# LukasHaas/PIGEON

Hardware: AMD Instinct MI355X
Metric: images/sec end-to-end (ViT+head+refine), 4x336x336 (higher is better)
Workload: dtype f16

## Files before the change

### include/pigeon_hip.h

```cpp
#ifndef PIGEON_HIP_H
#define PIGEON_HIP_H

#include <stddef.h>
#include <stdint.h>

#ifdef __cplusplus
extern "C" {
#endif

#define PG_OK            0
#define PG_EINVAL       -1
#define PG_ENOMEM       -2
#define PG_EHIP         -3
#define PG_ESTATE       -4

#define PG_DTYPE_F32     0
#define PG_DTYPE_BF16    1
#define PG_DTYPE_F16     2
#define PG_DTYPE_F64     3
#define PG_DTYPE_U8      4

#define PG_ABI_VERSION   7

const char* pg_last_error(void);
// ... 97 lines not shown
                        float* tol, int32_t* code, void* stream);

int pg_refine_certainty_bank(const pg_bank* bank, const float* q, int B, int P, const int64_t* cand, const float* cand_prob, int k,
                             int topk, int n_eval, const float* scratch12, const float* W, int C, const float* beta,
                             const float* wstats, float temperature, const int32_t* refined, const int32_t* choice,
                             float* tol, int32_t* code, float bank_sigma, void* stream);

int pg_requeue_append(const float* head_tol, const float* refine_tol, const int32_t* refine_code, int B, float thr, int force_all,
                      int64_t dst_base, int64_t flushed, int64_t cap, int64_t* counters, int64_t* slot_dst, int32_t* row_slot,
                      uint8_t* certain, int32_t* cause, void* stream);
int pg_rows_to_slots(const void* src, int64_t row_bytes, const int32_t* row_slot, int B, void* dst, void* stream);
int pg_requeue_take(const int64_t* slot_dst, int64_t cap, int64_t head, int n_valid, int n_pad, int64_t* dst_out, void* stream);
int pg_scatter_rows(const void* src, int64_t row_bytes, const int64_t* dst_row, int n, void* dst, int64_t dst_rows,
                    int64_t remap_wb, int64_t remap_b, int64_t remap_off, void* stream);
int pg_head_wstats(const float* W, int C, const float* beta, float* out2, void* stream);

int pg_embedding_debias(float* emb, int64_t n, int dim, const float* bias, void* stream);

int pg_token_attribution(const float* hidden, int n_images, int P, const float* W, int C, const int64_t* cells,
                         const int64_t* against, int K, float* out, void* stream);

typedef struct pg_prep pg_prep;
int pg_prep_create(pg_prep** out, int device, int in_h, int in_w);
int pg_prep_destroy(pg_prep* h);
int pg_prep_geometry(const pg_prep* h, int32_t* out6);
int pg_prep_workspace_bytes(const pg_prep* h, int n_images, size_t* bytes);
int pg_prep_norm_lut(float out[768]);
int pg_prep_forward(pg_prep* h, const void* images_u8, int n_images, void* out, int out_dtype, void* workspace,
                    size_t workspace_bytes, void* stream);

// ... 110 lines not shown
int pg_op_gemm16_ld(int dtype, const void* A, int64_t lda, const void* W, int64_t ldw, const float* bias, void* out,
                    int64_t ldc, int M, int N, int K, int epi, float qscale, int qcols, const float* aux,
                    int variant, void* stream);
int pg_op_rowstat_cast(const float* x, void* x16, int dtype, float* rowstat, int64_t rows, float eps, void* stream);
int pg_op_gemm16_resid_stat(int dtype, const void* A, int64_t lda, const void* W, int64_t ldw, const float* bias, float* X,
                            int64_t ldc, void* x16, int64_t ldx, float* statpart, int M, int N, int K, int variant, void* stream);
int pg_op_rowstat_finalize(const float* statpart, int slots, float* rowstat, int64_t rows, float eps, void* stream);
int pg_op_gemm16_ln(int dtype, const void* A, int64_t lda, const void* W, int64_t ldw, const float* bias, const float* colsum,
                    const float* rowstat, void* out, int64_t ldc, int M, int N, int K, int epi, float qscale, int qcols,
                    int variant, void* stream);
int pg_op_layernorm(const float* x, const float* gamma, const float* beta, void* y, int out_dtype,
                    int64_t rows, float eps, void* stream);
int pg_op_attention(int dtype, const void* qkv, void* out, int n_images, void* stream);
int pg_op_im2col(const void* pixels, int pix_dtype, void* out, int out_dtype, int n_images, void* stream);
int pg_op_token_mean(const float* x, float* out, int n_images, void* stream);
int pg_op_cast_f32(const float* x, void* y, int out_dtype, int64_t n, void* stream);
int pg_op_preln(float* x, const float* cls, const float* pos0, const float* gamma, const float* beta, int64_t rows, float eps,
                void* x16, int x16_dtype, float* rowstat, void* stream);
int pg_op_gemm16_parts(int dtype, const void* A, int64_t lda, const void* W, int64_t ldw, const float* bias, float* parts,
                       int M, int N, int Kp, int S, void* stream);
int pg_op_x3_split(const float* x, void* y3, int64_t rows, int cols, int gelu, void* stream);
int pg_op_x3_layernorm(const float* x, const float* gamma, const float* beta, void* y3, int64_t rows, float eps, void* stream);
int pg_op_attention_f32(const float* qkv, float* out, int n_images, void* stream);
int pg_op_attention_x3(const float* qkv, void* out3, int n_images, void* stream);
int pg_op_x3_im2col(const void* pixels, int pix_dtype, void* out3, int n_images, void* stream);
int pg_op_sum_parts(const float* parts, int S, int64_t part_elems, float* dst, int64_t n, int resid, void* stream);

#ifdef __cplusplus
}
#endif
// ... 2 lines not shown
```

### pigeon_amd/_lib.py

```python
from __future__ import annotations

import ctypes as C
import os

_HERE = os.path.dirname(os.path.abspath(__file__))
LIB_PATH = os.environ.get("PIGEON_HIP_LIB") or os.path.join(_HERE, "libpigeon_hip.so")

PG_DTYPE_F32, PG_DTYPE_BF16, PG_DTYPE_F16, PG_DTYPE_F64, PG_DTYPE_U8 = 0, 1, 2, 3, 4
EPI_QKV, EPI_GELU, EPI_RESID, EPI_PATCH, EPI_F32, EPI_RESID_STAT, EPI_QKV_LN, EPI_GELU_LN, EPI_GELU_X3 = 0, 1, 2, 3, 4, 5, 6, 7, 8
PROF_CLASSES = ["gemm_qkv", "gemm_out", "gemm_fc1", "gemm_fc2", "gemm_patch", "attention", "layernorm",
                "im2col", "token_mean"]


class PigeonHipError(RuntimeError):
    pass


class VitCfg(C.Structure):
    _fields_ = [("layers", C.c_int32), ("image_size", C.c_int32), ("patch", C.c_int32), ("hidden", C.c_int32),
                ("heads", C.c_int32), ("mlp", C.c_int32), ("ln_eps", C.c_float), ("max_chunk", C.c_int32),
                ("mma_dtype", C.c_int32), ("precise", C.c_int32)]


class Bank(C.Structure):
# ... 19 lines not shown
PREP_ITEM_BYTES = 80
assert C.sizeof(PrepItem) == PREP_ITEM_BYTES


class JpegInfo(C.Structure):
    _fields_ = [("reason", C.c_int32), ("height", C.c_int32), ("width", C.c_int32), ("ncomp", C.c_int32), ("hs", C.c_int32),
                ("vs", C.c_int32), ("reserved", C.c_int32 * 2)]


class JpegItem(C.Structure):
    _fields_ = [("rgb_off", C.c_uint64), ("coef_off", C.c_uint64 * 3), ("plane_off", C.c_uint64 * 3), ("height", C.c_int32),
                ("width", C.c_int32), ("ncomp", C.c_int32), ("hs", C.c_int32), ("vs", C.c_int32), ("bw", C.c_int32 * 3),
                ("bh", C.c_int32 * 3), ("qsel", C.c_int32 * 3), ("reserved", C.c_int32 * 4), ("qt", (C.c_uint16 * 64) * 4)]


JPEG_ITEM_BYTES = 640
assert C.sizeof(JpegItem) == JPEG_ITEM_BYTES and C.sizeof(JpegInfo) == 32
JPEG_REASONS = ("ok", "not_jpeg", "progressive", "lossless", "hierarchical", "arithmetic", "precision", "components", "colorspace",
                "sampling", "multiscan", "dnl", "size", "malformed")


_P, _I, _I64, _F, _D, _SZ = C.c_void_p, C.c_int, C.c_int64, C.c_float, C.c_double, C.c_size_t
SIGNATURES = {
    "pg_last_error": (C.c_char_p, []),
    "pg_abi_version": (_I, []),
    "pg_device_count": (_I, []),
    "pg_vit_create": (_I, [C.POINTER(_P), _I, C.POINTER(VitCfg)]),
    "pg_vit_load_weight": (_I, [_P, C.c_char_p, _P, _I, C.POINTER(_I64), _I]),
    "pg_vit_finalize": (_I, [_P]),
    "pg_vit_workspace_bytes": (_I, [_P, _I, C.POINTER(_SZ)]),
# ... 59 lines not shown
    "pg_region_plan": (_I, [C.POINTER(RegionBankStruct), C.POINTER(C.c_int32)]),
    "pg_tune_region_wave_edges": (_I, [_I]),
    "pg_head_forward": (_I, [_P, _I, _I, _P, _P, _P, _I, _I, _P, _P, _P, _P, _P, _P]),
    "pg_head_margin": (_I, [_P, _I, _I, _P, _I, _P, _P, _P, _P, _P]),
    "pg_head_certainty": (_I, [_P, _I, _I, _P, _I, _P, _P, _I, _P, _P, _P, _P, _P, _P, _P]),
    "pg_aux_heads_forward": (_I, [_P, _I, _I, _P, _P, _I, _I, _I, _P, _P, _P, _P, _P, _P, _P]),
    "pg_refine_forward": (_I, [C.POINTER(Bank), _P, _I, _I, _P, _P, _P, _I, _I, _F, _D, _P, _P, _P, _P, _P]),
    "pg_refine_forward_ex": (_I, [C.POINTER(Bank), _P, _I, _I, _P, _P, _P, _I, _I, _I, _F, _D, _P, _P, _P, _P, _P, _P]),
    "pg_refine_certainty": (_I, [C.POINTER(Bank), _P, _I, _I, _P, _P, _I, _I, _I, _P, _P, _I, _P, _P, _F, _P, _P, _P, _P, _P]),
    "pg_refine_certainty_bank": (_I, [C.POINTER(Bank), _P, _I, _I, _P, _P, _I, _I, _I, _P, _P, _I, _P, _P, _F, _P, _P, _P, _P, _F, _P]),
    "pg_requeue_append": (_I, [_P, _P, _P, _I, _F, _I, _I64, _I64, _I64, _P, _P, _P, _P, _P, _P]),
    "pg_rows_to_slots": (_I, [_P, _I64, _P, _I, _P, _P]),
    "pg_requeue_take": (_I, [_P, _I64, _I64, _I, _I, _P, _P]),
    "pg_scatter_rows": (_I, [_P, _I64, _P, _I, _P, _I64, _I64, _I64, _I64, _P]),
    "pg_head_wstats": (_I, [_P, _I, _P, _P, _P]),
    "pg_embedding_debias": (_I, [_P, _I64, _I, _P, _P]),
    "pg_token_attribution": (_I, [_P, _I, _I, _P, _I, _P, _P, _I, _P, _P]),
    "pg_op_gemm16": (_I, [_I, _P, _I64, _P, _P, _P, _I64, _I, _I, _I, _I, _F, _I, _P, _I, _P]),
    "pg_op_gemm16_ld": (_I, [_I, _P, _I64, _P, _I64, _P, _P, _I64, _I, _I, _I, _I, _F, _I, _P, _I, _P]),
    "pg_op_rowstat_cast": (_I, [_P, _P, _I, _P, _I64, _F, _P]),
    "pg_op_gemm16_resid_stat": (_I, [_I, _P, _I64, _P, _I64, _P, _P, _I64, _P, _I64, _P, _I, _I, _I, _I, _P]),
    "pg_op_rowstat_finalize": (_I, [_P, _I, _P, _I64, _F, _P]),
    "pg_op_gemm16_ln": (_I, [_I, _P, _I64, _P, _I64, _P, _P, _P, _P, _I64, _I, _I, _I, _I, _F, _I, _I, _P]),
    "pg_op_layernorm": (_I, [_P, _P, _P, _P, _I, _I64, _F, _P]),
    "pg_op_attention": (_I, [_I, _P, _P, _I, _P]),
    "pg_op_im2col": (_I, [_P, _I, _P, _I, _I, _P]),
    "pg_op_token_mean": (_I, [_P, _P, _I, _P]),
    "pg_op_cast_f32": (_I, [_P, _P, _I, _I64, _P]),
    "pg_op_gemm16_parts": (_I, [_I, _P, _I64, _P, _I64, _P, _P, _I, _I, _I, _I, _P]),
    "pg_op_x3_split": (_I, [_P, _P, _I64, _I, _I, _P]),
    "pg_op_x3_layernorm": (_I, [_P, _P, _P, _P, _I64, _F, _P]),
    "pg_op_attention_f32": (_I, [_P, _P, _I, _P]),
    "pg_op_attention_x3": (_I, [_P, _P, _I, _P]),
    "pg_op_x3_im2col": (_I, [_P, _I, _P, _I, _P]),
    "pg_op_sum_parts": (_I, [_P, _I, _I64, _P, _I64, _I, _P]),
    "pg_op_preln": (_I, [_P, _P, _P, _P, _P, _I64, _F, _P, _I, _P, _P]),
    "pg_vit_precise_plan": (_I, [_I, C.POINTER(C.c_int32)]),
}

_lib = None


# ... 32 lines not shown
```

### pigeon_amd/csrc/abi.hip

```cpp
#include "pigeon_internal.h"
#include <cstdarg>
#include <cstdio>

static thread_local char g_err[512] = "";

void pg_set_error(const char* fmt, ...) {
    va_list ap;
    va_start(ap, fmt);
    vsnprintf(g_err, sizeof(g_err), fmt, ap);
    va_end(ap);
}
int pg_check_launch(const char* what) {
    hipError_t e = hipGetLastError();
    if (e != hipSuccess) { pg_set_error("launch of %s failed: %s", what, hipGetErrorString(e)); return PG_EHIP; }
    return PG_OK;
}

extern "C" const char* pg_last_error(void) { return g_err; }
extern "C" int pg_abi_version(void) { return PG_ABI_VERSION; }
extern "C" int pg_device_count(void) {
    int n = 0;
    hipError_t e = hipGetDeviceCount(&n);
    if (e != hipSuccess) { pg_set_error("hipGetDeviceCount: %s", hipGetErrorString(e)); return PG_EHIP; }
    return n;
// ... 44 lines not shown
extern "C" int pg_op_attention(int dtype, const void* qkv, void* out, int n_images, void* stream) {
    if (!qkv || !out) { pg_set_error("op_attention: null argument"); return PG_EINVAL; }
    return pg_attention_launch(dtype, qkv, out, n_images, (hipStream_t)stream);
}
extern "C" int pg_op_im2col(const void* pixels, int pix_dtype, void* out, int out_dtype, int n_images, void* stream) {
    if (!pixels || !out) { pg_set_error("op_im2col: null argument"); return PG_EINVAL; }
    if (out_dtype == PG_DTYPE_U8) { pg_set_error("op_im2col: PG_DTYPE_U8 is a pixel dtype, not an output dtype"); return PG_EINVAL; }
    const float* lut = nullptr;
    if (pix_dtype == PG_DTYPE_U8 && n_images > 0) { const int rc = pg_norm_lut_device(&lut); if (rc) return rc; }
    return pg_im2col_launch(pixels, pix_dtype, out, out_dtype, n_images, (hipStream_t)stream, lut);
}
extern "C" int pg_op_token_mean(const float* x, float* out, int n_images, void* stream) {
    if (!x || !out) { pg_set_error("op_token_mean: null argument"); return PG_EINVAL; }
    return pg_token_mean_launch(x, out, n_images, (hipStream_t)stream);
}
extern "C" int pg_op_cast_f32(const float* x, void* y, int out_dtype, int64_t n, void* stream) {
    if (!x || !y) { pg_set_error("op_cast_f32: null argument"); return PG_EINVAL; }
    return pg_cast_f32_launch(x, y, out_dtype, n, (hipStream_t)stream);
}

extern "C" int pg_op_gemm16_parts(int dtype, const void* A, int64_t lda, const void* W, int64_t ldw, const float* bias, float* parts,
                                  int M, int N, int Kp, int S, void* stream) {
    if (!A || !W || !parts) { pg_set_error("op_gemm16_parts: null argument"); return PG_EINVAL; }
    if (S < 1 || S > 8) { pg_set_error("op_gemm16_parts: 1 <= S <= 8"); return PG_EINVAL; }
    PgGemmExtra ex;
    ex.parts = S; ex.a_part = Kp; ex.w_part = Kp; ex.c_part = (int64_t)M * N;
    return pg_gemm_launch(dtype, A, lda, W, ldw, bias, parts, N, M, N, Kp, EPI_F32, 1.f, 0, nullptr, PG_GEMM_V_PP, (hipStream_t)stream, &ex);
}

extern "C" int pg_op_x3_split(const float* x, void* y3, int64_t rows, int cols, int gelu, void* stream) {
// ... 33 lines not shown
```

### pigeon_amd/csrc/comm.hip

```cpp
#include "pigeon_internal.h"

#include <dlfcn.h>
#include <unistd.h>
#include <cstdio>
#include <cstdlib>
#include <cstring>
#include <rccl/rccl.h>

namespace {

struct Rccl {
    void* lib = nullptr;
    ncclResult_t (*GetUniqueId)(ncclUniqueId*) = nullptr;
    ncclResult_t (*CommInitRank)(ncclComm_t*, int, ncclUniqueId, int) = nullptr;
    ncclResult_t (*CommDestroy)(ncclComm_t) = nullptr;
    ncclResult_t (*CommCount)(const ncclComm_t, int*) = nullptr;
    ncclResult_t (*AllGather)(const void*, void*, size_t, ncclDataType_t, ncclComm_t, hipStream_t) = nullptr;
    ncclResult_t (*GroupStart)() = nullptr;
    ncclResult_t (*GroupEnd)() = nullptr;
    const char* (*GetErrorString)(ncclResult_t) = nullptr;
    ncclResult_t (*GetVersion)(int*) = nullptr;
};

Rccl* rccl() {
// ... 85 lines not shown
    if (!R) return PG_EHIP;
    pg_comm* c = (pg_comm*)comm;
    PG_NCCL(R->AllGather(send, recv, bytes_per_rank, ncclInt8, c->comm, (hipStream_t)stream));
    return PG_OK;
}

extern "C" int pg_allgather_many(void* comm, int count, const void* const* send, void* const* recv, const size_t* bytes_per_rank,
                                 void* stream) {
    if (!comm || count < 0 || (count > 0 && (!send || !recv || !bytes_per_rank))) { pg_set_error("allgather_many: bad argument"); return PG_EINVAL; }
    if (count == 0) return PG_OK;
    Rccl* R = rccl();
    if (!R) return PG_EHIP;
    pg_comm* c = (pg_comm*)comm;
    for (int i = 0; i < count; ++i)
        if (bytes_per_rank[i] && (!send[i] || !recv[i])) { pg_set_error("allgather_many: null buffer %d", i); return PG_EINVAL; }
    PG_NCCL(R->GroupStart());
    ncclResult_t first = ncclSuccess;
    for (int i = 0; i < count; ++i) {
        if (!bytes_per_rank[i]) continue;
        const ncclResult_t e = R->AllGather(send[i], recv[i], bytes_per_rank[i], ncclInt8, c->comm, (hipStream_t)stream);
        if (e != ncclSuccess && first == ncclSuccess) first = e;
    }
    const ncclResult_t e2 = R->GroupEnd();
    if (first != ncclSuccess) { pg_set_error("ncclAllGather (grouped) failed: %s", R->GetErrorString(first)); return PG_EHIP; }
    if (e2 != ncclSuccess) { pg_set_error("ncclGroupEnd failed: %s", R->GetErrorString(e2)); return PG_EHIP; }
    return PG_OK;
}

extern "C" int pg_comm_destroy(void* comm) {
    if (!comm) return PG_OK;
// ... 15 lines not shown
```

### pigeon_amd/csrc/head.hip

```cpp
#include "common.h"
#include "pigeon_internal.h"
#include "certainty_common.h"
#include <cfloat>

#define HT 64
#define HK 32

__global__ __launch_bounds__(256) void head_logits_kernel(const float* __restrict__ emb, int B, int P,
                                                          const float* __restrict__ W, const float* __restrict__ bias,
                                                          int C, float* __restrict__ logits) {
    __shared__ float As[HK][HT + 1];
    __shared__ float Ws[HK][HT + 1];
    const int tid = threadIdx.x;
    const int c0 = blockIdx.x * HT, b0 = blockIdx.y * HT;
    const int tx = tid & 15, ty = tid >> 4;
    float acc[4][4];
#pragma unroll
    for (int i = 0; i < 4; ++i)
#pragma unroll
        for (int j = 0; j < 4; ++j) acc[i][j] = 0.f;
    const float invP = 1.0f / (float)P;
    for (int k0 = 0; k0 < VIT_HIDDEN; k0 += HK) {
#pragma unroll
        for (int i = 0; i < 8; ++i) {
            const int idx = tid + i * 256;
// ... 20 lines not shown
#pragma unroll
                for (int j = 0; j < 4; ++j) acc[i][j] = fmaf(a[i], w[j], acc[i][j]);
        }
        __syncthreads();
    }
#pragma unroll
    for (int i = 0; i < 4; ++i) {
        const int b = b0 + ty * 4 + i;
        if (b >= B) continue;
#pragma unroll
        for (int j = 0; j < 4; ++j) {
            const int c = c0 + tx * 4 + j;
            if (c < C) logits[(int64_t)b * C + c] = acc[i][j] + bias[c];
        }
    }
}

struct ValIdx { float v; int i; };
__device__ __forceinline__ ValIdx block_argbest(ValIdx x, ValIdx* red ) {
#pragma unroll
    for (int o = 32; o >= 1; o >>= 1) {
        const float ov = __shfl_xor(x.v, o, 64);
        const int oi = __shfl_xor(x.i, o, 64);
        if (better(ov, oi, x.v, x.i)) { x.v = ov; x.i = oi; }
    }
    const int wave = threadIdx.x >> 6;
    __syncthreads();
    if ((threadIdx.x & 63) == 0) red[wave] = x;
    __syncthreads();
    ValIdx r = red[0];
// ... 50 lines not shown
        if (GLOBAL) __threadfence_block();
        __syncthreads();
    }
}

extern "C" int pg_head_forward(const float* emb, int B, int P, const float* W, const float* bias,
                               const double* centroids, int C, int k, float* logits, float* topk_val,
                               int64_t* topk_idx, int64_t* argmax, double* pred_llh, void* stream) {
    hipStream_t s = (hipStream_t)stream;
    if (B < 0) { pg_set_error("head: B = %d", B); return PG_EINVAL; }
    if (B == 0) return PG_OK;
    if (!emb || !W || !bias || !centroids || !logits || !topk_val || !topk_idx || !argmax || !pred_llh) {
        pg_set_error("head: null pointer argument"); return PG_EINVAL;
    }
    if (P < 1 || C < 1 || k < 1 || k > C) { pg_set_error("head: bad P=%d C=%d k=%d", P, C, k); return PG_EINVAL; }
    const size_t lds = (size_t)C * sizeof(float);
    const bool big = lds > 150 * 1024;
    dim3 g1((C + HT - 1) / HT, (B + HT - 1) / HT);
    hipLaunchKernelGGL(head_logits_kernel, g1, dim3(256), 0, s, emb, B, P, W, bias, C, logits);
    int rc = pg_check_launch("head_logits");
    if (rc) return rc;
    if (big) {
        float* scratch = nullptr;
        PG_HIP(hipMallocAsync((void**)&scratch, (size_t)B * C * sizeof(float), s));
        hipLaunchKernelGGL(head_row_kernel<true>, dim3(B), dim3(256), 0, s, logits, C, k, centroids, topk_val, topk_idx, argmax, pred_llh, scratch);
        rc = pg_check_launch("head_row (large C)");
        (void)hipFreeAsync(scratch, s);
        return rc;
    }
    static size_t attr_lds = 0;
    if (lds > attr_lds) {
        PG_HIP(hipFuncSetAttribute((const void*)head_row_kernel<false>, hipFuncAttributeMaxDynamicSharedMemorySize, (int)lds));
        attr_lds = lds;
    }
    hipLaunchKernelGGL(head_row_kernel<false>, dim3(B), dim3(256), lds, s, logits, C, k, centroids, topk_val, topk_idx, argmax, pred_llh,
// ... 63 lines not shown
```

### pigeon_amd/csrc/pigeon_internal.h

```cpp
#pragma once
#include <hip/hip_runtime.h>
#include <stdint.h>
#include "../../include/pigeon_hip.h"

enum { EPI_QKV = 0, EPI_GELU = 1, EPI_RESID = 2, EPI_PATCH = 3, EPI_F32 = 4, EPI_RESID_STAT = 5, EPI_QKV_LN = 6, EPI_GELU_LN = 7,
       EPI_GELU_X3 = 8 };

struct PgGemmExtra {
    const float* colsum = nullptr;
    const float* rowstat = nullptr;
    void* x16 = nullptr;
    int64_t ldx = 0;
    float* statpart = nullptr;
    int64_t stat_rows = 0;
    int parts = 1;
    int64_t a_part = 0, w_part = 0, c_part = 0;
};

void pg_set_error(const char* fmt, ...) __attribute__((format(printf, 1, 2)));
int pg_check_launch(const char* what);
int pg_default_gemm_variant();
int pg_gemm_grid_cus();
int pg_gemm_raster_gn();
unsigned long long pg_tune_epoch();
// ... 16 lines not shown
void pg_fingerprint_host(const void* data, size_t bytes, uint64_t seed, uint64_t out[2]);

#define PG_NORM_LUT_SIZE (3 * 256)
void pg_norm_lut_fill(float* lut);
int pg_norm_lut_device(const float** lut);

int pg_gemm_launch(int dtype, const void* A, int64_t lda, const void* W, int64_t ldw, const float* bias, void* out, int64_t ldc,
                   int M, int N, int K, int epi, float qscale, int qcols, const float* aux, int variant,
                   hipStream_t s, const PgGemmExtra* extra = nullptr);
int pg_layernorm_launch(const float* x, const float* gamma, const float* beta, void* y, int out_dtype,
                        int64_t rows, float eps, hipStream_t s);
int pg_preln_launch(float* x, const float* cls, const float* pos0, const float* gamma, const float* beta,
                    int64_t rows, float eps, hipStream_t s, void* x16 = nullptr, int x16_dtype = 0, float* rowstat = nullptr);
int pg_im2col_launch(const void* pixels, int pix_dtype, void* out, int out_dtype, int n_images, hipStream_t s, const float* norm_lut = nullptr);
int pg_token_mean_launch(const float* x, float* out, int n_images, hipStream_t s);
int pg_cast_f32_launch(const float* x, void* y, int out_dtype, int64_t n, hipStream_t s);
int pg_rowstat_cast_launch(const float* x, void* x16, int out_dtype, float* rowstat, int64_t rows, float eps, hipStream_t s);
int pg_rowstat_finalize_launch(const float* statpart, int slots, float* rowstat, int64_t rows, float eps, hipStream_t s,
                               unsigned long long* alarm = nullptr, float alarm_sumsq = 0.f);
int pg_count_sat16_launch(const void* buf, int64_t rows, int cols, int64_t ld, int dtype, unsigned long long* counter, hipStream_t s);
int pg_attention_launch(int dtype, const void* qkv, void* out, int n_images, hipStream_t s);
int pg_x3_ln_launch(const float* x, const float* gamma, const float* beta, void* y3, int64_t rows, float eps, hipStream_t s);
int pg_x3_split_launch(const float* x, void* y3, int64_t rows, int C, int gelu, hipStream_t s);
int pg_x3_im2col_launch(const void* pixels, int pix_dtype, void* out3, int n_images, hipStream_t s, const float* norm_lut = nullptr);
int pg_attention_f32_launch(const float* qkv, float* out, int n_images, hipStream_t s);
bool pg_attention_x3out_available();
int pg_attention_x3out_launch(const float* qkv, void* out3, int n_images, hipStream_t s);
int pg_sum_parts_launch(const float* parts, int S, int64_t part_elems, float* dst, int64_t n, int resid, hipStream_t s);
```

### pigeon_amd/csrc/requeue.hip

```cpp
#include "common.h"
#include "pigeon_internal.h"

namespace {

__global__ void __launch_bounds__(256)
requeue_append_kernel(const float* __restrict__ head_tol, const float* __restrict__ refine_tol, const int32_t* __restrict__ refine_code,
                      int B, float thr, int force_all, int64_t dst_base, int64_t flushed, int64_t cap,
                      int64_t* __restrict__ counters, int64_t* __restrict__ slot_dst, int32_t* __restrict__ row_slot,
                      uint8_t* __restrict__ certain, int32_t* __restrict__ cause) {
    __shared__ int wave_cnt[4];
    __shared__ int64_t s_app, s_drop;
    const int tid = threadIdx.x, lane = tid & 63, wv = tid >> 6;
    if (tid == 0) { s_app = counters ? counters[0] : 0; s_drop = counters ? counters[1] : 0; }
    __syncthreads();
    for (int base = 0; base < B; base += 256) {
        const int r = base + tid;
        bool flag = false;
        int why = 0;
        if (r < B) {
            const bool h_unc = force_all || !(head_tol[r] > thr);
            const bool r_unc = refine_tol ? !(refine_tol[r] > thr) : false;
            flag = h_unc || r_unc;
            why = h_unc ? 1 : (r_unc ? (refine_code ? refine_code[r] : 2) : 0);
            if (r_unc && !h_unc && why == 0) why = 2;
// ... 82 lines not shown
        const f32x4 v = *(const f32x4*)(row + i * 256 + lane * 4);
        n2 = fmaf(v[0], v[0], fmaf(v[1], v[1], fmaf(v[2], v[2], fmaf(v[3], v[3], n2))));
        if (beta) {
            const f32x4 b = *(const f32x4*)(beta + i * 256 + lane * 4);
            wb = fmaf(v[0], b[0], fmaf(v[1], b[1], fmaf(v[2], b[2], fmaf(v[3], b[3], wb))));
        }
    }
    n2 = wave_sum(n2);
    wb = wave_sum(wb);
    if (lane == 0) {
        atomicMax(out + 0, __float_as_uint(sqrtf(n2)));
        atomicMax(out + 1, __float_as_uint(fabsf(wb)));
    }
}

int vec_bytes(const void* a, const void* b, int64_t row_bytes) {
    const uintptr_t al = (uintptr_t)a | (uintptr_t)b | (uintptr_t)row_bytes;
    return (al & 15) == 0 ? 16 : (al & 7) == 0 ? 8 : (al & 3) == 0 ? 4 : 1;
}
dim3 row_grid(int64_t row_bytes, int vb, int rows) {
    int64_t chunks = (row_bytes / vb + 256 * 8 - 1) / (256 * 8);
    if (chunks < 1) chunks = 1;
    if (chunks > 256) chunks = 256;
    return dim3((unsigned)chunks, (unsigned)rows, 1);
}

}

extern "C" int pg_requeue_append(const float* head_tol, const float* refine_tol, const int32_t* refine_code, int B, float thr,
                                 int force_all, int64_t dst_base, int64_t flushed, int64_t cap, int64_t* counters, int64_t* slot_dst,
// ... 26 lines not shown
                               int64_t remap_wb, int64_t remap_b, int64_t remap_off, void* stream) {
    if (n < 0 || row_bytes < 0 || dst_rows < 0) { pg_set_error("scatter_rows: bad size"); return PG_EINVAL; }
    if (n == 0 || row_bytes == 0) return PG_OK;
    if (!src || !dst_row || !dst) { pg_set_error("scatter_rows: null argument"); return PG_EINVAL; }
    if (n > 65535) { pg_set_error("scatter_rows: n = %d rows exceed the launch grid (65535)", n); return PG_EINVAL; }
    const int vb = vec_bytes(src, dst, row_bytes);
    const dim3 g = row_grid(row_bytes, vb, n);
    hipStream_t s = (hipStream_t)stream;
#define PG_SCATTER(V) hipLaunchKernelGGL(scatter_rows_kernel<V>, g, dim3(256), 0, s, (const char*)src, row_bytes, dst_row, (char*)dst, \
                                         dst_rows, remap_wb, remap_b, remap_off)
    if (vb == 16) PG_SCATTER(uint4); else if (vb == 8) PG_SCATTER(uint2); else if (vb == 4) PG_SCATTER(uint32_t); else PG_SCATTER(uint8_t);
#undef PG_SCATTER
    return pg_check_launch("scatter_rows_kernel");
}

extern "C" int pg_requeue_take(const int64_t* slot_dst, int64_t cap, int64_t head, int n_valid, int n_pad, int64_t* dst_out, void* stream) {
    if (n_pad < 0 || n_valid < 0 || n_valid > n_pad || cap <= 0 || head < 0) { pg_set_error("requeue_take: bad argument"); return PG_EINVAL; }
    if (n_pad == 0) return PG_OK;
    if (!slot_dst || !dst_out) { pg_set_error("requeue_take: null argument"); return PG_EINVAL; }
    hipLaunchKernelGGL(requeue_take_kernel, dim3((n_pad + 255) / 256), dim3(256), 0, (hipStream_t)stream, slot_dst, cap, head, n_valid, n_pad, dst_out);
    return pg_check_launch("requeue_take_kernel");
}

extern "C" int pg_head_wstats(const float* W, int C, const float* beta, float* out2, void* stream) {
    if (C < 0) { pg_set_error("head_wstats: C = %d", C); return PG_EINVAL; }
    if (!out2 || (C > 0 && !W)) { pg_set_error("head_wstats: null argument"); return PG_EINVAL; }
    hipStream_t s = (hipStream_t)stream;
    PG_HIP(hipMemsetAsync(out2, 0, 2 * sizeof(float), s));
    if (C == 0) return PG_OK;
    hipLaunchKernelGGL(head_wstats_kernel, dim3((C + 3) / 4), dim3(256), 0, s, W, C, beta, (unsigned int*)out2);
// ... 3 lines not shown
```

### pigeon_amd/deferred.py

```python
from __future__ import annotations

from collections import deque
from typing import Dict, List, NamedTuple, Optional

import torch

from .utils import TopK


AUX_KEYS = ('aux_preds', 'aux_cls', 'aux_tol', 'aux_code')


class Col(NamedTuple):
    name: str
    where: str
    src: str
    when: str = 'always'
    dtype: Optional[torch.dtype] = None
    tail: tuple = ()


COLUMNS = (
    *(Col(k, 'ring', 'state') for k in ('embedding', 'topk_indices', 'topk_values', 'preds_LLH', 'preds_geocell')),
    Col('index', 'ring', 'index', dtype=torch.int64),
# ... 90 lines not shown
        self.q_pixels = torch.zeros((self.cap,) + tuple(px_rows.shape[1:]), dtype=px_rows.dtype, device=px_rows.device)
        self.slot_dst = torch.zeros((self.cap,), dtype=torch.int64, device=px_rows.device)
        self._true_cap = torch.ones((self.cap,), dtype=torch.bool, device=px_rows.device)
        self.px_shape = (tuple(px_rows.shape[1:]), px_rows.dtype)

    def _mark(self, m):
        if m is None:
            return
        if self.dev.type == 'cuda':
            ev = torch.cuda.Event(enable_timing=True)
            ev.record()
            m.append(ev)
        else:
            import time
            m.append(time.perf_counter())

    def _bank_kw(self) -> dict:
        if getattr(self.refiner, 'bank_rel_tol', 0.0) > 0:
            return {'kappa': self.model.certainty.kappa}
        return {}

    @torch.no_grad()
    def submit(self, pixel_values=None, embedding=None, index=None, meta=None, pixel_bytes=None) -> List[dict]:
        model, comm, ops = self.model, self.comm, self.ops
        marks = [] if self.marks is not None else None
        settled = []
        if self.dev is None:
            self.dev = model.cell_layer.weight.device
        self._mark(marks)
        st = model.encode_head(pixel_values, embedding) if pixel_bytes is None else model.encode_head(pixel_values, embedding, pixel_bytes=pixel_bytes)
# ... 17 lines not shown
        if self.ring is None:
            self._alloc(st, b)
        rank, B, WB = comm.rank, self.B, self.WB
        step = self.n_submitted
        slot = step % self.R
        if any(r['slot'] == slot for r in self.pending):
            raise RuntimeError('DeferredExact: result ring overrun (max_lag too large for the ring)')
        gbase, lbase = slot * WB, slot * B
        dev = self.dev
        if index is None:
            index = self._arange[:b] if rank == 0 else self._arange[:b] + rank * b
        index = index.to(dev)
        exact_tier = bool(st.get('exact_tier', False))
        thr = st['thr']
        new = dict(st, index=index)
        for k, buf in self.local.items():
            if k in st:
                buf[lbase:lbase + b].copy_(st[k])
        ring = self.ring
        slab = lambda k: ring[k][gbase:gbase + comm.world_size * b]
        own = slice(gbase + rank * b, gbase + (rank + 1) * b)
        self._mark(marks)
        comm.gather_many([new[k] for k in self.gather1], out=[slab(k) for k in self.gather1])
        self._mark(marks)
        rtol = rcode = None
        W_head = model.cell_layer.weight.data
        if self.refiner is not None:
            new['refined_LLH'], new['refined_geocell'], rtol, rcode, self.boundary_checked = self.refiner.forward_certain(
                ring['embedding'][own], ring['preds_LLH'][own], ring['topk_indices'][own], ring['topk_values'][own], W_head,
                st['wstats'], st.get('drift'), **self._bank_kw())
            new.update(refine_tol=rtol, refine_code=rcode)
            for k in self.local_refiner:
                self.local[k][lbase:lbase + b].copy_(new[k])
        wants_queue = bool(getattr(model, 'exact_top1', False)) and px is not None
        if wants_queue:
            px_rows = px.reshape((b, -1)).contiguous()
            if self.q_pixels is None or self.px_shape != (tuple(px_rows.shape[1:]), px_rows.dtype):
                if self.q_pixels is not None:
                    settled = settled + self.flush()
                    self.counters.zero_()
                    self.flushed = [0] * comm.world_size
                    self._prev_appended = [0] * comm.world_size
                self._alloc_queue(px_rows)
        if can_fix:
            certain, cause, row_slot = ops.requeue_append(st['tol'], rtol, rcode, thr, False, dst_base=gbase + rank * b,
                                                          flushed=self.flushed[rank], cap=self.cap, counters=self.counters,
                                                          slot_dst=self.slot_dst)
            ops.rows_to_slots(px_rows, row_slot, self.q_pixels)
# ... 133 lines not shown
    def exact_pass_ms(self, entries=None) -> List[float]:
        out = []
        for f in (self.flush_log if entries is None else entries):
            sp = f.get('span')
            if sp:
                out.append((sp[1] - sp[0]) * 1e3 if isinstance(sp[0], float) else sp[0].elapsed_time(sp[1]))
        return out

    def _emit(self, rec: dict) -> dict:
        if 'ready' in rec:
            return rec['ready']
        b = rec['b']
        gbase, lbase = rec['slot'] * self.WB, rec['slot'] * self.B
        queued = [a - p for a, p in zip(rec['appended'], self._prev_appended)]
        self._prev_appended = rec['appended']
        return self._result({k: v[gbase:gbase + self.comm.world_size * b].clone() for k, v in self.ring.items()},
                            {k: v[lbase:lbase + b].clone() for k, v in self.local.items()}, b, queued, rec['step'], rec['meta'])

    def check_nothing_dropped(self) -> int:
        return int(self.counters[1].item()) if self.ring is not None else 0


def round_quantum(px_rows: torch.Tensor, tokens: int = 577, panel_rows: int = 256, n_tiles: int = 4) -> int:
    if px_rows.device.type != 'cuda':
        return 0
    cus = torch.cuda.get_device_properties(px_rows.device).multi_processor_count
    images = (cus // n_tiles) * panel_rows // tokens
    views = max(1, int(px_rows.shape[1]) // (3 * 336 * 336))
    return max(1, images // views)


def as_model_output(model, res: dict, labels=None, labels_clf=None, labels_multi_task=None, labels_climate=None, labels_month=None):
# ... 7 lines not shown
```

### pigeon_amd/hip_ops.py

```python
from __future__ import annotations

import ctypes as C
from typing import Dict, Optional

import torch

from . import _lib
from ._lib import Bank, VitCfg, check, load

TOKENS, HIDDEN, MLP, PATCHES, KPAD = 577, 1024, 4096, 576, 640


def _p(t: Optional[torch.Tensor]):
    return C.c_void_p(0) if t is None else C.c_void_p(t.data_ptr())


def _stream():
    return C.c_void_p(torch.cuda.current_stream().cuda_stream)


_T16 = {torch.float16: _lib.PG_DTYPE_F16, torch.bfloat16: _lib.PG_DTYPE_BF16}
_PIXDT = {torch.float32: _lib.PG_DTYPE_F32, torch.float16: _lib.PG_DTYPE_F16, torch.bfloat16: _lib.PG_DTYPE_BF16}
_PIXIN = {**_PIXDT, torch.uint8: _lib.PG_DTYPE_U8}
_PREP_OUT = {torch.float32: _lib.PG_DTYPE_F32, torch.float16: _lib.PG_DTYPE_F16, torch.uint8: _lib.PG_DTYPE_U8}
# ... 883 lines not shown

def scatter_rows(src: torch.Tensor, dst_row: torch.Tensor, dst: torch.Tensor, remap=None) -> None:
    _dev(src); _dev(dst); _dev(dst_row, torch.int64)
    n = src.shape[0]
    _shape(dst_row, "dst_row", n)
    if src.dtype != dst.dtype or tuple(src.shape[1:]) != tuple(dst.shape[1:]):
        raise _lib.PigeonHipError(f"scatter_rows: rows of {src.dtype} {tuple(src.shape[1:])} into {dst.dtype} {tuple(dst.shape[1:])}")
    rb = 1
    for d in src.shape[1:]:
        rb *= int(d)
    rb *= src.element_size()
    wb, b, off = remap if remap is not None else (0, 0, 0)
    check(load().pg_scatter_rows(_p(src), rb, _p(dst_row), n, _p(dst), dst.shape[0], int(wb), int(b), int(off), _stream()), "pg_scatter_rows")


def x3_split(x: torch.Tensor, gelu: bool = False) -> torch.Tensor:
    _dev(x, torch.float32)
    rows, cols = x.shape
    y = torch.empty((rows, 3 * cols), dtype=torch.float16, device=x.device)
    check(load().pg_op_x3_split(_p(x), _p(y), rows, cols, 1 if gelu else 0, _stream()), "pg_op_x3_split")
    return y


def gemm16_parts(A: torch.Tensor, W: torch.Tensor, bias: Optional[torch.Tensor], S: int) -> torch.Tensor:
    _dev(A); _dev(W)
    if W.dtype != A.dtype or A.shape[1] != W.shape[1] or A.shape[1] % S:
        raise _lib.PigeonHipError("gemm16_parts: A and W must share dtype and a K' divisible by S")
    M, Kt = A.shape
    N = W.shape[0]
    out = torch.empty((S, M, N), dtype=torch.float32, device=A.device)
# ... 216 lines not shown
```

Baseline: 2507.

## Rewrite head logits as mean-then-GEMM and batch small copies into one kernel

The head logits kernel now first reduces embeddings over views into a mean buffer, then runs a double-buffered, register-tiled FP32 GEMM with a small-batch tile variant. The old kernel is kept as a reference op. Separately, the per-column copy_ calls in the deferred pipeline and the single-rank allgather are replaced by one segmented copy kernel, cutting launch and host overhead. This adds a hipMallocAsync per head call, a new 16-byte alignment requirement on emb and W, and inline asm FMAs.

```diff
diff --git a/include/pigeon_hip.h b/include/pigeon_hip.h
--- a/include/pigeon_hip.h
+++ b/include/pigeon_hip.h
@@ -135,6 +135,16 @@
 int pg_scatter_rows(const void* src, int64_t row_bytes, const int64_t* dst_row, int n, void* dst, int64_t dst_rows,
                     int64_t remap_wb, int64_t remap_b, int64_t remap_off, void* stream);
 int pg_head_wstats(const float* W, int C, const float* beta, float* out2, void* stream);
+
+#define PG_COPY_MAX_SEGS 64
+typedef struct pg_copy_seg {
+    const void* src;
+    void*       dst;
+    uint64_t    bytes;
+    int32_t     fill;
+    int32_t     reserved;
+} pg_copy_seg;
+int pg_copy_segments(const pg_copy_seg* segs, int n, void* stream);
 
 int pg_embedding_debias(float* emb, int64_t n, int dim, const float* bias, void* stream);
 
@@ -275,6 +285,7 @@
 int pg_op_attention(int dtype, const void* qkv, void* out, int n_images, void* stream);
 int pg_op_im2col(const void* pixels, int pix_dtype, void* out, int out_dtype, int n_images, void* stream);
 int pg_op_token_mean(const float* x, float* out, int n_images, void* stream);
+int pg_op_head_logits_ref(const float* emb, int B, int P, const float* W, const float* bias, int C, float* logits, void* stream);
 int pg_op_cast_f32(const float* x, void* y, int out_dtype, int64_t n, void* stream);
 int pg_op_preln(float* x, const float* cls, const float* pos0, const float* gamma, const float* beta, int64_t rows, float eps,
                 void* x16, int x16_dtype, float* rowstat, void* stream);
diff --git a/pigeon_amd/_lib.py b/pigeon_amd/_lib.py
--- a/pigeon_amd/_lib.py
+++ b/pigeon_amd/_lib.py
@@ -57,6 +57,11 @@
                 ("bh", C.c_int32 * 3), ("qsel", C.c_int32 * 3), ("reserved", C.c_int32 * 4), ("qt", (C.c_uint16 * 64) * 4)]
 
 
+class CopySeg(C.Structure):
+    _fields_ = [("src", C.c_void_p), ("dst", C.c_void_p), ("bytes", C.c_uint64), ("fill", C.c_int32), ("reserved", C.c_int32)]
+
+
+COPY_MAX_SEGS = 64
 JPEG_ITEM_BYTES = 640
 assert C.sizeof(JpegItem) == JPEG_ITEM_BYTES and C.sizeof(JpegInfo) == 32
 JPEG_REASONS = ("ok", "not_jpeg", "progressive", "lossless", "hierarchical", "arithmetic", "precision", "components", "colorspace",
@@ -146,6 +151,7 @@
     "pg_requeue_take": (_I, [_P, _I64, _I64, _I, _I, _P, _P]),
     "pg_scatter_rows": (_I, [_P, _I64, _P, _I, _P, _I64, _I64, _I64, _I64, _P]),
     "pg_head_wstats": (_I, [_P, _I, _P, _P, _P]),
+    "pg_copy_segments": (_I, [C.POINTER(CopySeg), _I, _P]),
     "pg_embedding_debias": (_I, [_P, _I64, _I, _P, _P]),
     "pg_token_attribution": (_I, [_P, _I, _I, _P, _I, _P, _P, _I, _P, _P]),
     "pg_op_gemm16": (_I, [_I, _P, _I64, _P, _P, _P, _I64, _I, _I, _I, _I, _F, _I, _P, _I, _P]),
@@ -158,6 +164,7 @@
     "pg_op_attention": (_I, [_I, _P, _P, _I, _P]),
     "pg_op_im2col": (_I, [_P, _I, _P, _I, _I, _P]),
     "pg_op_token_mean": (_I, [_P, _P, _I, _P]),
+    "pg_op_head_logits_ref": (_I, [_P, _I, _I, _P, _P, _I, _P, _P]),
     "pg_op_cast_f32": (_I, [_P, _P, _I, _I64, _P]),
     "pg_op_gemm16_parts": (_I, [_I, _P, _I64, _P, _I64, _P, _P, _I, _I, _I, _I, _P]),
     "pg_op_x3_split": (_I, [_P, _P, _I64, _I, _I, _P]),
diff --git a/pigeon_amd/csrc/abi.hip b/pigeon_amd/csrc/abi.hip
--- a/pigeon_amd/csrc/abi.hip
+++ b/pigeon_amd/csrc/abi.hip
@@ -82,6 +82,12 @@
     if (!x || !out) { pg_set_error("op_token_mean: null argument"); return PG_EINVAL; }
     return pg_token_mean_launch(x, out, n_images, (hipStream_t)stream);
 }
+extern "C" int pg_op_head_logits_ref(const float* emb, int B, int P, const float* W, const float* bias, int C, float* logits, void* stream) {
+    if (B < 0 || P < 1 || C < 1) { pg_set_error("op_head_logits_ref: bad B=%d P=%d C=%d", B, P, C); return PG_EINVAL; }
+    if (B == 0) return PG_OK;
+    if (!emb || !W || !bias || !logits) { pg_set_error("op_head_logits_ref: null argument"); return PG_EINVAL; }
+    return pg_head_logits_ref_launch(emb, B, P, W, bias, C, logits, (hipStream_t)stream);
+}
 extern "C" int pg_op_cast_f32(const float* x, void* y, int out_dtype, int64_t n, void* stream) {
     if (!x || !y) { pg_set_error("op_cast_f32: null argument"); return PG_EINVAL; }
     return pg_cast_f32_launch(x, y, out_dtype, n, (hipStream_t)stream);
diff --git a/pigeon_amd/csrc/comm.hip b/pigeon_amd/csrc/comm.hip
--- a/pigeon_amd/csrc/comm.hip
+++ b/pigeon_amd/csrc/comm.hip
@@ -123,6 +123,19 @@
     pg_comm* c = (pg_comm*)comm;
     for (int i = 0; i < count; ++i)
         if (bytes_per_rank[i] && (!send[i] || !recv[i])) { pg_set_error("allgather_many: null buffer %d", i); return PG_EINVAL; }
+    if (c->nranks == 1) {
+        pg_copy_seg segs[PG_COPY_MAX_SEGS];
+        int m = 0;
+        for (int i = 0; i < count; ++i) {
+            if (bytes_per_rank[i] && send[i] != recv[i]) segs[m++] = pg_copy_seg{send[i], recv[i], (uint64_t)bytes_per_rank[i], 0, 0};
+            if (m == PG_COPY_MAX_SEGS || (i == count - 1 && m > 0)) {
+                const int rc = pg_copy_segments(segs, m, stream);
+                if (rc) return rc;
+                m = 0;
+            }
+        }
+        return PG_OK;
+    }
     PG_NCCL(R->GroupStart());
     ncclResult_t first = ncclSuccess;
     for (int i = 0; i < count; ++i) {
diff --git a/pigeon_amd/csrc/head.hip b/pigeon_amd/csrc/head.hip
--- a/pigeon_amd/csrc/head.hip
+++ b/pigeon_amd/csrc/head.hip
@@ -6,9 +6,9 @@
 #define HT 64
 #define HK 32
 
-__global__ __launch_bounds__(256) void head_logits_kernel(const float* __restrict__ emb, int B, int P,
-                                                          const float* __restrict__ W, const float* __restrict__ bias,
-                                                          int C, float* __restrict__ logits) {
+__global__ __launch_bounds__(256) void head_logits_ref_kernel(const float* __restrict__ emb, int B, int P,
+                                                              const float* __restrict__ W, const float* __restrict__ bias,
+                                                              int C, float* __restrict__ logits) {
     __shared__ float As[HK][HT + 1];
     __shared__ float Ws[HK][HT + 1];
     const int tid = threadIdx.x;
@@ -59,6 +59,164 @@
             if (c < C) logits[(int64_t)b * C + c] = acc[i][j] + bias[c];
         }
     }
+}
+
+__global__ __launch_bounds__(256) void head_mean_kernel(const float* __restrict__ emb, int P, float* __restrict__ mean) {
+    const int b = blockIdx.x, k = threadIdx.x * 4;
+    const float* e = emb + ((int64_t)b * P) * VIT_HIDDEN + k;
+    const float invP = 1.0f / (float)P;
+    f32x4 a = {0.f, 0.f, 0.f, 0.f};
+    for (int p = 0; p < P; ++p) {
+        const f32x4 v = *(const f32x4*)(e + (int64_t)p * VIT_HIDDEN);
+#pragma unroll
+        for (int i = 0; i < 4; ++i) a[i] += v[i];
+    }
+#pragma unroll
+    for (int i = 0; i < 4; ++i) a[i] *= invP;
+    *(f32x4*)(mean + (int64_t)b * VIT_HIDDEN + k) = a;
+}
+
+typedef float f32x2 __attribute__((ext_vector_type(2)));
+
+__device__ __forceinline__ void fmac(float& acc, float a, float w) { asm("v_fmac_f32_e32 %0, %1, %2" : "+v"(acc) : "v"(a), "v"(w)); }
+
+template <int BM, int BN, int TN, int BK>
+__global__ __launch_bounds__((BM / 4) * (BN / TN)) void head_logits_kernel(const float* __restrict__ mean, int B,
+                                                                            const float* __restrict__ W, const float* __restrict__ bias,
+                                                                            int C, int row_tiles, float* __restrict__ logits) {
+    constexpr int NT = (BM / 4) * (BN / TN), Q = BK / 4;
+    constexpr int LA = BM * Q / NT, LW = BN * Q / NT;
+    static_assert(BM * Q % NT == 0 && BN * Q % NT == 0 && VIT_HIDDEN % BK == 0 && (TN == 8 || TN == 2), "tile shape");
+    __shared__ __attribute__((aligned(16))) float As[2][BK][BM + 4];
+    __shared__ __attribute__((aligned(16))) float Ws[2][BK][BN + 4];
+    const int tid = threadIdx.x;
+    const int group = 8 * row_tiles, rr = blockIdx.x % group;
+    const int ct = (blockIdx.x / group) * 8 + (rr & 7), bt = rr >> 3;
+    const int c0 = ct * BN, b0 = bt * BM;
+    if (c0 >= C) return;
+    const int tx = tid % (BN / TN), ty = tid / (BN / TN);
+    float acc[4][TN];
+#pragma unroll
+    for (int i = 0; i < 4; ++i)
+#pragma unroll
+        for (int j = 0; j < TN; ++j) acc[i][j] = 0.f;
+    f32x4 ra[LA], rw[LW];
+    const f32x4 zero = {0.f, 0.f, 0.f, 0.f};
+    auto fetch = [&](int k0) {
+#pragma unroll
+        for (int i = 0; i < LA; ++i) {
+            const int idx = tid + i * NT, r = idx / Q, q = idx % Q;
+            ra[i] = (b0 + r < B) ? *(const f32x4*)(mean + (int64_t)(b0 + r) * VIT_HIDDEN + k0 + q * 4) : zero;
+        }
+#pragma unroll
+        for (int i = 0; i < LW; ++i) {
+            const int idx = tid + i * NT, r = idx / Q, q = idx % Q;
+            rw[i] = (c0 + r < C) ? *(const f32x4*)(W + (int64_t)(c0 + r) * VIT_HIDDEN + k0 + q * 4) : zero;
+        }
+    };
+    auto stage = [&](int buf) {
+#pragma unroll
+        for (int i = 0; i < LA; ++i) {
+            const int idx = tid + i * NT, r = idx / Q, q = idx % Q;
+#pragma unroll
+            for (int e = 0; e < 4; ++e) As[buf][q * 4 + e][r] = ra[i][e];
+        }
+#pragma unroll
+        for (int i = 0; i < LW; ++i) {
+            const int idx = tid + i * NT, r = idx / Q, q = idx % Q;
+#pragma unroll
+            for (int e = 0; e < 4; ++e) Ws[buf][q * 4 + e][r] = rw[i][e];
+        }
+    };
+    constexpr int KC = 4;
+    static_assert(BK % (2 * KC) == 0, "K step");
+    struct Chunk { f32x4 a[KC]; float w[KC][TN]; };
+    Chunk ping, pong;
+    auto load = [&](Chunk& ch, int buf, int kk) {
+#pragma unroll
+        for (int u = 0; u < KC; ++u) {
+            ch.a[u] = *(const f32x4*)&As[buf][kk + u][ty * 4];
+            if constexpr (TN == 8) {
+                const f32x4 w0 = *(const f32x4*)&Ws[buf][kk + u][tx * 8], w1 = *(const f32x4*)&Ws[buf][kk + u][tx * 8 + 4];
+#pragma unroll
+                for (int j = 0; j < 4; ++j) { ch.w[u][j] = w0[j]; ch.w[u][4 + j] = w1[j]; }
+            } else {
+                const f32x2 w0 = *(const f32x2*)&Ws[buf][kk + u][tx * 2];
+                ch.w[u][0] = w0[0]; ch.w[u][1] = w0[1];
+            }
+        }
+    };
+    auto fma_chunk = [&](const Chunk& ch) {
+#pragma unroll
+        for (int u = 0; u < KC; ++u)
+#pragma unroll
+            for (int i = 0; i < 4; ++i)
+#pragma unroll
+                for (int j = 0; j < TN; ++j) fmac(acc[i][j], ch.a[u][i], ch.w[u][j]);
+    };
+    fetch(0);
+    stage(0);
+    __syncthreads();
+    constexpr int STEPS = VIT_HIDDEN / BK;
+    for (int s = 0; s < STEPS; ++s) {
+        const int buf = s & 1;
+        if (s + 1 < STEPS) fetch((s + 1) * BK);
+        load(ping, buf, 0);
+#pragma unroll 1
+        for (int kk = 0; kk < BK - 2 * KC; kk += 2 * KC) {
+            load(pong, buf, kk + KC);
+            fma_chunk(ping);
+            load(ping, buf, kk + 2 * KC);
+            fma_chunk(pong);
+        }
+        load(pong, buf, BK - KC);
+        fma_chunk(ping);
+        fma_chunk(pong);
+        if (s + 1 < STEPS) stage(buf ^ 1);
+        __syncthreads();
+    }
+#pragma unroll
+    for (int i = 0; i < 4; ++i) {
+        const int b = b0 + ty * 4 + i;
+        if (b >= B) continue;
+#pragma unroll
+        for (int j = 0; j < TN; ++j) {
+            const int c = c0 + tx * TN + j;
+            if (c < C) logits[(int64_t)b * C + c] = acc[i][j] + bias[c];
+        }
+    }
+}
+
+struct HeadLogitsPlan { bool small; int row_tiles, col_tiles, threads; };
+static HeadLogitsPlan head_logits_plan(int B, int C) {
+    HeadLogitsPlan p;
+    p.small = B <= 16;
+    const int bm = p.small ? 16 : 64, bn = p.small ? 32 : 64;
+    p.row_tiles = (B + bm - 1) / bm;
+    p.col_tiles = (C + bn - 1) / bn;
+    p.threads = p.small ? 64 : 128;
+    return p;
+}
+
+static int head_logits_launch(const float* emb, int B, int P, const float* W, const float* bias, int C, float* logits, hipStream_t s) {
+    float* mean = nullptr;
+    PG_HIP(hipMallocAsync((void**)&mean, (size_t)B * VIT_HIDDEN * sizeof(float), s));
+    hipLaunchKernelGGL(head_mean_kernel, dim3(B), dim3(256), 0, s, emb, P, mean);
+    int rc = pg_check_launch("head_mean");
+    if (!rc) {
+        const HeadLogitsPlan p = head_logits_plan(B, C);
+        const dim3 grid((unsigned)((p.col_tiles + 7) / 8 * 8 * p.row_tiles));
+        if (p.small) hipLaunchKernelGGL((head_logits_kernel<16, 32, 2, 64>), grid, dim3(p.threads), 0, s, mean, B, W, bias, C, p.row_tiles, logits);
+        else hipLaunchKernelGGL((head_logits_kernel<64, 64, 8, 32>), grid, dim3(p.threads), 0, s, mean, B, W, bias, C, p.row_tiles, logits);
+        rc = pg_check_launch("head_logits");
+    }
+    (void)hipFreeAsync(mean, s);
+    return rc;
+}
+
+int pg_head_logits_ref_launch(const float* emb, int B, int P, const float* W, const float* bias, int C, float* logits, hipStream_t s) {
+    hipLaunchKernelGGL(head_logits_ref_kernel, dim3((C + HT - 1) / HT, (B + HT - 1) / HT), dim3(256), 0, s, emb, B, P, W, bias, C, logits);
+    return pg_check_launch("head_logits_ref");
 }
 
 struct ValIdx { float v; int i; };
@@ -139,11 +297,10 @@
         pg_set_error("head: null pointer argument"); return PG_EINVAL;
     }
     if (P < 1 || C < 1 || k < 1 || k > C) { pg_set_error("head: bad P=%d C=%d k=%d", P, C, k); return PG_EINVAL; }
+    if ((((uintptr_t)emb | (uintptr_t)W) & 15) != 0) { pg_set_error("head: emb and W must be 16-byte aligned"); return PG_EINVAL; }
     const size_t lds = (size_t)C * sizeof(float);
     const bool big = lds > 150 * 1024;
-    dim3 g1((C + HT - 1) / HT, (B + HT - 1) / HT);
-    hipLaunchKernelGGL(head_logits_kernel, g1, dim3(256), 0, s, emb, B, P, W, bias, C, logits);
-    int rc = pg_check_launch("head_logits");
+    int rc = head_logits_launch(emb, B, P, W, bias, C, logits, s);
     if (rc) return rc;
     if (big) {
         float* scratch = nullptr;
diff --git a/pigeon_amd/csrc/pigeon_internal.h b/pigeon_amd/csrc/pigeon_internal.h
--- a/pigeon_amd/csrc/pigeon_internal.h
+++ b/pigeon_amd/csrc/pigeon_internal.h
@@ -54,6 +54,7 @@
                     int64_t rows, float eps, hipStream_t s, void* x16 = nullptr, int x16_dtype = 0, float* rowstat = nullptr);
 int pg_im2col_launch(const void* pixels, int pix_dtype, void* out, int out_dtype, int n_images, hipStream_t s, const float* norm_lut = nullptr);
 int pg_token_mean_launch(const float* x, float* out, int n_images, hipStream_t s);
+int pg_head_logits_ref_launch(const float* emb, int B, int P, const float* W, const float* bias, int C, float* logits, hipStream_t s);
 int pg_cast_f32_launch(const float* x, void* y, int out_dtype, int64_t n, hipStream_t s);
 int pg_rowstat_cast_launch(const float* x, void* x16, int out_dtype, float* rowstat, int64_t rows, float eps, hipStream_t s);
 int pg_rowstat_finalize_launch(const float* statpart, int slots, float* rowstat, int64_t rows, float eps, hipStream_t s,
diff --git a/pigeon_amd/csrc/requeue.hip b/pigeon_amd/csrc/requeue.hip
--- a/pigeon_amd/csrc/requeue.hip
+++ b/pigeon_amd/csrc/requeue.hip
@@ -1,5 +1,6 @@
 #include "common.h"
 #include "pigeon_internal.h"
+#include <cstring>
 
 namespace {
 
@@ -120,6 +121,37 @@
     }
 }
 
+constexpr int64_t SEG_CHUNK = 65536;
+struct SegTable {
+    pg_copy_seg seg[PG_COPY_MAX_SEGS];
+    int32_t first[PG_COPY_MAX_SEGS + 1];
+};
+
+__global__ void __launch_bounds__(256) copy_segments_kernel(const SegTable t, int n) {
+    const int blk = blockIdx.x, tid = threadIdx.x;
+    int lo = 0, hi = n;
+    while (hi - lo > 1) {
+        const int mid = (lo + hi) >> 1;
+        if (t.first[mid] <= blk) lo = mid; else hi = mid;
+    }
+    const int64_t off = (int64_t)(blk - t.first[lo]) * SEG_CHUNK;
+    const int64_t left = (int64_t)t.seg[lo].bytes - off;
+    const int len = (int)(left < SEG_CHUNK ? left : SEG_CHUNK);
+    const unsigned char* src = t.seg[lo].src ? (const unsigned char*)t.seg[lo].src + off : nullptr;
+    unsigned char* dst = (unsigned char*)t.seg[lo].dst + off;
+    const unsigned int f = (unsigned int)(t.seg[lo].fill & 0xff) * 0x01010101u;
+    const bool vec = (((uintptr_t)dst | (uintptr_t)src) & 15) == 0;
+    const int n16 = vec ? len >> 4 : 0;
+    if (src) {
+        for (int i = tid; i < n16; i += 256) ((uint4*)dst)[i] = ((const uint4*)src)[i];
+        for (int i = (n16 << 4) + tid; i < len; i += 256) dst[i] = src[i];
+    } else {
+        const uint4 v = make_uint4(f, f, f, f);
+        for (int i = tid; i < n16; i += 256) ((uint4*)dst)[i] = v;
+        for (int i = (n16 << 4) + tid; i < len; i += 256) dst[i] = (unsigned char)f;
+    }
+}
+
 int vec_bytes(const void* a, const void* b, int64_t row_bytes) {
     const uintptr_t al = (uintptr_t)a | (uintptr_t)b | (uintptr_t)row_bytes;
     return (al & 15) == 0 ? 16 : (al & 7) == 0 ? 8 : (al & 3) == 0 ? 4 : 1;
@@ -176,6 +208,27 @@
     return pg_check_launch("scatter_rows_kernel");
 }
 
+extern "C" int pg_copy_segments(const pg_copy_seg* segs, int n, void* stream) {
+    if (n < 0 || n > PG_COPY_MAX_SEGS) { pg_set_error("copy_segments: n = %d segments (0..%d)", n, PG_COPY_MAX_SEGS); return PG_EINVAL; }
+    if (n == 0) return PG_OK;
+    if (!segs) { pg_set_error("copy_segments: null table"); return PG_EINVAL; }
+    SegTable t;
+    memset(&t, 0, sizeof(t));
+    int64_t blocks = 0;
+    for (int i = 0; i < n; ++i) {
+        if (segs[i].bytes && !segs[i].dst) { pg_set_error("copy_segments: segment %d has no destination", i); return PG_EINVAL; }
+        t.seg[i] = segs[i];
+        t.first[i] = (int32_t)blocks;
+        const uint64_t chunks = segs[i].bytes / (uint64_t)SEG_CHUNK + (segs[i].bytes % (uint64_t)SEG_CHUNK != 0);
+        blocks = chunks > 0x7fffffffull ? (int64_t)0x80000000ll : blocks + (int64_t)chunks;
+        if (blocks > 0x7fffffff) { pg_set_error("copy_segments: more than 2^31 chunks"); return PG_EINVAL; }
+    }
+    for (int i = n; i <= PG_COPY_MAX_SEGS; ++i) t.first[i] = (int32_t)blocks;
+    if (blocks == 0) return PG_OK;
+    hipLaunchKernelGGL(copy_segments_kernel, dim3((unsigned)blocks), dim3(256), 0, (hipStream_t)stream, t, n);
+    return pg_check_launch("copy_segments_kernel");
+}
+
 extern "C" int pg_requeue_take(const int64_t* slot_dst, int64_t cap, int64_t head, int n_valid, int n_pad, int64_t* dst_out, void* stream) {
     if (n_pad < 0 || n_valid < 0 || n_valid > n_pad || cap <= 0 || head < 0) { pg_set_error("requeue_take: bad argument"); return PG_EINVAL; }
     if (n_pad == 0) return PG_OK;
diff --git a/pigeon_amd/deferred.py b/pigeon_amd/deferred.py
--- a/pigeon_amd/deferred.py
+++ b/pigeon_amd/deferred.py
@@ -128,6 +128,16 @@
         else:
             import time
             m.append(time.perf_counter())
+
+    def _copy_columns(self, pairs):
+        many = getattr(self.ops, 'copy_segments', None)
+        plain = [(s, d) for s, d in pairs if many is not None and d.is_cuda and s.is_cuda and s.device == d.device
+                 and s.dtype == d.dtype and s.shape == d.shape]
+        if plain:
+            many(plain)
+        for s, d in pairs:
+            if not any(d is q for _, q in plain):
+                d.copy_(s)
 
     def _bank_kw(self) -> dict:
         if getattr(self.refiner, 'bank_rel_tol', 0.0) > 0:
@@ -175,9 +185,7 @@
         exact_tier = bool(st.get('exact_tier', False))
         thr = st['thr']
         new = dict(st, index=index)
-        for k, buf in self.local.items():
-            if k in st:
-                buf[lbase:lbase + b].copy_(st[k])
+        self._copy_columns([(st[k], buf[lbase:lbase + b]) for k, buf in self.local.items() if k in st])
         ring = self.ring
         slab = lambda k: ring[k][gbase:gbase + comm.world_size * b]
         own = slice(gbase + rank * b, gbase + (rank + 1) * b)
@@ -191,8 +199,7 @@
                 ring['embedding'][own], ring['preds_LLH'][own], ring['topk_indices'][own], ring['topk_values'][own], W_head,
                 st['wstats'], st.get('drift'), **self._bank_kw())
             new.update(refine_tol=rtol, refine_code=rcode)
-            for k in self.local_refiner:
-                self.local[k][lbase:lbase + b].copy_(new[k])
+            self._copy_columns([(new[k], self.local[k][lbase:lbase + b]) for k in self.local_refiner])
         wants_queue = bool(getattr(model, 'exact_top1', False)) and px is not None
         if wants_queue:
             px_rows = px.reshape((b, -1)).contiguous()
@@ -356,8 +363,11 @@
         gbase, lbase = rec['slot'] * self.WB, rec['slot'] * self.B
         queued = [a - p for a, p in zip(rec['appended'], self._prev_appended)]
         self._prev_appended = rec['appended']
-        return self._result({k: v[gbase:gbase + self.comm.world_size * b].clone() for k, v in self.ring.items()},
-                            {k: v[lbase:lbase + b].clone() for k, v in self.local.items()}, b, queued, rec['step'], rec['meta'])
+        ring = {k: v[gbase:gbase + self.comm.world_size * b] for k, v in self.ring.items()}
+        local = {k: v[lbase:lbase + b] for k, v in self.local.items()}
+        out_ring, out_local = ({k: torch.empty_like(v) for k, v in d.items()} for d in (ring, local))
+        self._copy_columns([(v, out_ring[k]) for k, v in ring.items()] + [(v, out_local[k]) for k, v in local.items()])
+        return self._result(out_ring, out_local, b, queued, rec['step'], rec['meta'])
 
     def check_nothing_dropped(self) -> int:
         return int(self.counters[1].item()) if self.ring is not None else 0
diff --git a/pigeon_amd/hip_ops.py b/pigeon_amd/hip_ops.py
--- a/pigeon_amd/hip_ops.py
+++ b/pigeon_amd/hip_ops.py
@@ -921,6 +921,44 @@
     check(load().pg_scatter_rows(_p(src), rb, _p(dst_row), n, _p(dst), dst.shape[0], int(wb), int(b), int(off), _stream()), "pg_scatter_rows")
 
 
+def copy_segments(pairs) -> None:
+    segs = []
+    keep = []
+    for src, dst in pairs:
+        _dev(dst)
+        if not dst.is_contiguous():
+            raise _lib.PigeonHipError("copy_segments: destinations must be contiguous")
+        nbytes = dst.numel() * dst.element_size()
+        if isinstance(src, int):
+            if not 0 <= src <= 255:
+                raise _lib.PigeonHipError(f"copy_segments: fill byte {src}")
+            segs.append(_lib.CopySeg(None, dst.data_ptr(), nbytes, src, 0))
+            continue
+        _dev(src)
+        if src.dtype != dst.dtype or tuple(src.shape) != tuple(dst.shape) or src.device != dst.device:
+            raise _lib.PigeonHipError(f"copy_segments: {src.dtype} {tuple(src.shape)} on {src.device} into {dst.dtype} {tuple(dst.shape)} "
+                                      f"on {dst.device}")
+        src = src.contiguous()
+        keep.append(src)
+        segs.append(_lib.CopySeg(src.data_ptr(), dst.data_ptr(), nbytes, 0, 0))
+    stream = _stream() if segs else None
+    for i in range(0, len(segs), _lib.COPY_MAX_SEGS):
+        part = segs[i:i + _lib.COPY_MAX_SEGS]
+        check(load().pg_copy_segments((_lib.CopySeg * len(part))(*part), len(part), stream), "pg_copy_segments")
+
+
+def head_logits_ref(emb: torch.Tensor, W: torch.Tensor, bias: torch.Tensor) -> torch.Tensor:
+    _dev(emb, torch.float32); _dev(W, torch.float32); _dev(bias, torch.float32)
+    B = emb.shape[0]
+    P = emb.shape[1] if emb.dim() == 3 else 1
+    _shape(emb, "emb", *((B, P, HIDDEN) if emb.dim() == 3 else (B, HIDDEN)))
+    Cn = W.shape[0]
+    _shape(W, "W", Cn, HIDDEN); _shape(bias, "bias", Cn)
+    logits = torch.empty((B, Cn), dtype=torch.float32, device=emb.device)
+    check(load().pg_op_head_logits_ref(_p(emb), B, P, _p(W), _p(bias), Cn, _p(logits), _stream()), "pg_op_head_logits_ref")
+    return logits
+
+
 def x3_split(x: torch.Tensor, gelu: bool = False) -> torch.Tensor:
     _dev(x, torch.float32)
     rows, cols = x.shape
```

Result: no change. 2510 (median of 5 runs) (+0.1%).
